# oppo-us-research/PoP-Net

Measured on AMD Instinct MI355X. Metric: depth-frames/sec end-to-end (480x640), higher is better.
Workload: dtype bf16

## Files before the change

### popnet_amd/csrc/api.hip

```cpp
#pragma clang fp contract(off)
#include <cmath>
#include <cstdarg>
#include <cstdio>
#include <cstdlib>
#include <cstring>
#include "pn_internal.h"
#include "preproc_pixel.h"

template <typename TIN>
__global__ void preprocess_kernel(const TIN *__restrict__ depth, float *__restrict__ out, int B, int H, int W, int S,
                                  double scale_x, double scale_y, float dmax, float mean, float stdv) {
    const unsigned pix = blockIdx.x * blockDim.x + threadIdx.x;
    if (pix >= (unsigned)(S * S)) return;
    const int b = blockIdx.y;
    const int dy = (int)(pix / (unsigned)S);
    const int dx = (int)(pix - (unsigned)dy * (unsigned)S);
    const size_t gid = (size_t)b * S * S + pix;

    out[gid] = pn_preproc_pixel(depth + (size_t)b * H * W, H, W, dy, dx, scale_x, scale_y, dmax, mean, stdv);
}

PnSwitches pn_read_switches() {
    auto set = [](const char *name) { return getenv(name) != nullptr; };
    auto num = [](const char *name, int unset) { const char *e = getenv(name); return e ? atoi(e) : unset; };
    auto is = [](const char *name, const char *value) { const char *e = getenv(name); return e && !strcmp(e, value); };
    PnSwitches s;
    s.no_conv3 = set("POPNET_NO_CONV3");
    s.conv3_rpg8 = set("POPNET_CONV3_RPG8");
    s.conv3_pt14 = num("POPNET_CONV3_PT14", 0);
    s.conv3_nbuf2 = set("POPNET_CONV3_NBUF2");
    s.generic_c64_off = num("POPNET_GENERIC_C64", 1) == 0;
    if (set("POPNET_CONV4")) s.conv4 = num("POPNET_CONV4", 0) == 0 ? 0 : 1;
    s.no_mix = set("POPNET_NO_MIX");
    s.no_bblock = set("POPNET_NO_BBLOCK");
    s.bblock_x3 = num("POPNET_BBLOCK_X3", 0) != 0;
    s.bb64_static = set("POPNET_BB64_STATIC");
    s.bb64_halves = num("POPNET_BB64_HALVES", 1) == 2 ? 2 : 1;
    s.no_tailfuse = set("POPNET_NO_TAILFUSE");
    s.no_poolfuse = set("POPNET_NO_POOLFUSE");
    s.no_stempool = set("POPNET_NO_STEMPOOL");
    s.no_embed3 = set("POPNET_NO_EMBED3");
    s.train_x3_wide = set("POPNET_TRAIN_X3_WIDE");
    s.train_wgrad_novec = set("POPNET_TRAIN_WGRAD_NOVEC");
    s.trainx_one_stream = num("POPNET_TRAINX_STREAMS", 0) == 1;
    s.trainx_stem_handover = set("POPNET_TRAINX_STEM_HANDOVER");
    s.trainx_stem_gather = is("POPNET_TRAINX_STEM_FWD", "gather");
    s.trainx_stem_bn_separate = is("POPNET_TRAINX_STEM_BN", "separate");
    s.trainx_stem_depth = num("POPNET_TRAINX_STEM_DEPTH", 2);
    s.trainx_pack_gather = is("POPNET_TRAINX_PACK", "gather");
    s.trainx_legacy_wgrad = is("POPNET_TRAINX_WGRAD", "legacy");
    return s;
}

extern "C" {

int pn_abi_version(void) { return PN_ABI_VERSION; }
int pn_build_experiments(void) { return 0; }

pn_ctx *pn_create(int device_id) {
    pn_ctx *ctx = new pn_ctx();
    ctx->device = device_id;
    int ndev = 0;
    hipError_t e = hipGetDeviceCount(&ndev);
    if (e != hipSuccess || device_id < 0 || device_id >= ndev) {
        char buf[256];
        snprintf(buf, sizeof buf, "pn_create: device %d not available (%d devices, %s)", device_id, ndev,
                 hipGetErrorString(e));
        ctx->err = buf;
        ctx->device = -1;
        return ctx;
    }
    hipDeviceProp_t prop;
    if (hipGetDeviceProperties(&prop, device_id) == hipSuccess) ctx->num_cus = prop.multiProcessorCount;
    return ctx;
}

void pn_destroy(pn_ctx *ctx) {
    if (!ctx) return;
    if (ctx->parse_ws) (void)hipFree(ctx->parse_ws);
    pn_parse_big_free(ctx);
    if (ctx->train_ws) (void)hipFree(ctx->train_ws);
    for (void *p : ctx->train_ws_retired) (void)hipFree(p);
    for (auto &e : ctx->train_packs) (void)hipFree(e.buf);
    if (ctx->train_pack_table) (void)hipFree(ctx->train_pack_table);
    delete ctx;
}

}

int pn_set_error(pn_ctx *ctx, int code, const char *fmt, ...) {
    char buf[1024];
    va_list ap;
    va_start(ap, fmt);
    vsnprintf(buf, sizeof(buf), fmt, ap);
    va_end(ap);
    if (ctx) ctx->err = buf;
    return code;
}

extern "C" {

int pn_last_error(pn_ctx *ctx, char *buf, size_t buf_len) {
    if (!ctx) return 0;
    if (buf && buf_len) {
        size_t n = ctx->err.size() < buf_len - 1 ? ctx->err.size() : buf_len - 1;
        memcpy(buf, ctx->err.data(), n);
        buf[n] = 0;
    }
    return (int)ctx->err.size();
}

int pn_preprocess(pn_ctx *ctx, const void *depth_dev, int depth_dtype, int B, int H, int W, float *out_dev, int S,
                  float depth_max, float depth_mean, float depth_std, void *hip_stream) {
    if (!ctx) return PN_ERR_INVALID;
    if (ctx->device < 0) return pn_set_error(ctx, PN_ERR_STATE, "context has no device");
    if (!depth_dev || !out_dev || B < 1 || H < 2 || W < 2 || S < 1)
        return pn_set_error(ctx, PN_ERR_INVALID, "pn_preprocess: bad arguments");
    if (W == 2 * S && H == 2 * S)
        return pn_set_error(ctx, PN_ERR_UNSUPPORTED, "pn_preprocess: %dx%d -> %d is an exact 2x decimation, where cv2.resize(INTER_LINEAR) runs INTER_AREA instead: not built", W, H, S);
    const double inv_x = (double)S / (double)W, inv_y = (double)S / (double)H;
// ... 35 lines not shown
```

### popnet_amd/csrc/bb64_kernel.h

```cpp
#pragma once
#include "conv3_kernel.h"


#define BB_INQ (12 * 32 * 32)
#define BB_IN (4 * BB_INQ)
#define BB_MIDQ (10 * 32 * 32)
#define BB_MID (4 * BB_MIDQ)
#define BB_ASLOT 4096
#define BB_OFF_MID (2 * BB_IN)
#define BB_OFF_A (BB_OFF_MID + BB_MID)
#define BB_NSLOT 6
#define BB_LDS (BB_OFF_A + BB_NSLOT * BB_ASLOT)
#define BB_BIAS(cv, q) (BB_OFF_MID + (q) * BB_MIDQ + (((cv) + 1) * 32 + 30) * 32)

__host__ __device__ constexpr int bb_item_ks(int n, int PT, bool xch) { return !xch || n < 16 * PT ? n / PT : n - 16 * PT < 4 ? 16 + ((n - 16 * PT) >> 1) : 16 + ((n - 16 * PT) & 1); }
__host__ __device__ constexpr int bb_item_pt(int n, int PT, bool xch) { return !xch || n < 16 * PT ? n % PT : n - 16 * PT < 4 ? (n - 16 * PT) & 1 : (n - 16 * PT) >> 1; }

typedef __attribute__((ext_vector_type(2))) float f32x2;
typedef __attribute__((ext_vector_type(2))) __bf16 bf16x2;
typedef __attribute__((ext_vector_type(2))) short i16x2;
__device__ __forceinline__ unsigned bb_relu_pk(unsigned w) {
    return __builtin_bit_cast(unsigned, __builtin_elementwise_max(__builtin_bit_cast(i16x2, w), i16x2{0, 0}));
}

template <int HV>
__global__ __launch_bounds__((4 * HV + 4) * 64, 1) void bb64_kernel(const BBProblem P) {
    typedef __bf16 T;
    constexpr int CT = 4 / HV, NCW = 4 * HV, NP = CT / 2, PT1 = 5, PT2 = 4, KK = 9, BQ = 6;
    constexpr bool SPLIT = HV == 1;
    constexpr bool XCH = HV == 1;
    constexpr int NKO = XCH ? 16 : 18;
    constexpr int FILL1 = 7, FILL2 = 11;
    extern __shared__ __attribute__((aligned(16))) char smem[];
    const int tid = threadIdx.x;
    const int lane = tid & 63;
    const int wave = __builtin_amdgcn_readfirstlane(tid >> 6);
    const int c = lane & 15, q = lane >> 4;
    const int W = P.W, H = P.H;

    volatile int *s_tile = reinterpret_cast<volatile int *>(smem + BB_OFF_MID + 31 * 32);
    const bool dyn = P.tickets != nullptr;
    auto next_tile = [&](int t, int k) -> int { return dyn ? __builtin_amdgcn_readfirstlane(s_tile[(k + 1) & 3]) : t + (int)gridDim.x; };
    auto next_tile_raw = [&](int t, int k) -> int { return dyn ? s_tile[(k + 1) & 3] : t + (int)gridDim.x; };
    auto tile_geom = [&](int t, int &b, int &oy0, int &ox0, int &R, int &Wc) {
        b = t / P.tiles_per_img;
        const int rem = t - b * P.tiles_per_img;
        const int ty = rem / P.tiles_x, tx = rem - ty * P.tiles_x;
        oy0 = ty * 8; ox0 = tx * P.Wt;
        R = min(8, H - oy0); Wc = min(P.Wt, W - ox0);
    };

    if (wave >= NCW) {
        const int lw = wave - NCW;
        const unsigned lane16 = (unsigned)lane * 16u;
        int t = blockIdx.x;
        if (t >= P.ntiles) return;
        if (lw < 2) {
            const char *wsrc = (const char *)P.wpack + lw * 2048;
            auto dma_a = [&](int kstep) {
                pn_glds16_s<0>(wsrc + (size_t)kstep * BB_ASLOT, lane16, (unsigned)(BB_OFF_A + (kstep % BB_NSLOT) * BB_ASLOT) + (unsigned)__builtin_amdgcn_readfirstlane(lw * 2048));
                pn_glds16_s<0>(wsrc + (size_t)kstep * BB_ASLOT + 1024, lane16, (unsigned)(BB_OFF_A + (kstep % BB_NSLOT) * BB_ASLOT + 1024) + (unsigned)__builtin_amdgcn_readfirstlane(lw * 2048));
            };
            dma_a(0); dma_a(1); dma_a(2); dma_a(3);
            asm volatile("s_waitcnt vmcnt(0)\n\ts_barrier" ::: "memory");
            asm volatile("s_barrier" ::: "memory");
            for (int k = 0; t < P.ntiles; ++k) {
                const int tnx = next_tile_raw(t, k);
#pragma clang loop unroll(full)
                for (int p = 0; p < 18; ++p) {
                    dma_a((2 * p + 4) % 36);
                    dma_a((2 * p + 5) % 36);
                    asm volatile("s_waitcnt vmcnt(2)\n\ts_barrier" ::: "memory");
                    if (p == 8) asm volatile("s_barrier" ::: "memory");
                }
                asm volatile("s_barrier" ::: "memory");
                t = __builtin_amdgcn_readfirstlane(tnx);
            }
            asm volatile("s_waitcnt vmcnt(0)" ::: "memory");
            return;
        }
        auto dma_in = [&](int tt, int buf, int n) {
            int b, oy0, ox0, R, Wc;
            tile_geom(tt, b, oy0, ox0, R, Wc);
            const int qu = n / 12, row = n % 12;
            const int px = lane >> 1;
            const int iy = oy0 - 2 + row, ix = ox0 - 2 + px;
            const size_t frame_b = ((size_t)b * H * W * P.in_cs + P.in_coff) * 2;
            const bool inb = px < Wc + 4 && (unsigned)ix < (unsigned)W && (unsigned)iy < (unsigned)H;
            const unsigned off = inb ? (unsigned)((iy * W + ix) * P.in_cs * 2 + qu * 32 + (lane & 1) * 16) : P.in_zero_off - (unsigned)frame_b;
            pn_glds16_s<0>((const char *)P.in + frame_b, off, (unsigned)__builtin_amdgcn_readfirstlane(buf * BB_IN + qu * BB_INQ + row * 1024));
        };
        const int n0 = (lw - 2) * 24;
        const bool ticketer = dyn && lw == 2 && lane == 0;
        int ticket = 0;
        auto claim = [&]() -> int { return 2 * (int)gridDim.x + atomicAdd(P.tickets, 1); };
        if (ticketer) ticket = t + (int)gridDim.x;
#pragma unroll
        for (int j = 0; j < 24; ++j) dma_in(t, 0, n0 + j);
        asm volatile("s_waitcnt vmcnt(0)" ::: "memory");
        if (ticketer) s_tile[1] = ticket;
        asm volatile("s_waitcnt lgkmcnt(0)\n\ts_barrier" ::: "memory");
        asm volatile("s_barrier" ::: "memory");
        int cur = 0;
        for (int k = 0; t < P.ntiles; ++k) {
            const int tnx = next_tile(t, k);
            const int tn = tnx < P.ntiles ? tnx : t;
// ... 267 lines not shown
```

### popnet_amd/csrc/net_run.hip

```cpp
#include <algorithm>
#include <cstring>
#include "net_internal.h"

namespace pnnet {
int upload_net(pn_net *n) {
    pn_ctx *ctx = n->ctx;
    PN_HIP_CHECK(ctx, hipSetDevice(ctx->device));
    for (auto &b : n->bufs) {
        PN_HIP_CHECK(ctx, hipMalloc(&b.p, b.bytes + 2048));
        PN_HIP_CHECK(ctx, hipMemset(b.p, 0, b.bytes + 2048));
    }
    for (auto &im : n->images) {
        PN_HIP_CHECK(ctx, hipMalloc(&im.dev, im.bytes));
        if (im.host.empty()) PN_HIP_CHECK(ctx, hipMemset(im.dev, 0, im.bytes));
        else PN_HIP_CHECK(ctx, hipMemcpy(im.dev, im.host.data(), im.bytes, hipMemcpyHostToDevice));
    }
    PN_HIP_CHECK(ctx, hipDeviceSynchronize());
    return PN_OK;
}

void release_net(pn_net *n) {
    for (auto &b : n->bufs) if (b.p) (void)hipFree(b.p);
    for (auto &im : n->images) if (im.dev) (void)hipFree(im.dev);
    for (auto &r : n->prof) { (void)hipEventDestroy(r.a); (void)hipEventDestroy(r.b); }
// ... 81 lines not shown
        PN_HIP_CHECK(n->ctx, hipMemcpyAsync(n->dev(st.dev_probs), st.host_probs.data(), st.host_probs.size() * sizeof(ConvProblem),
                                            hipMemcpyHostToDevice, stream));
    }
    n->last_B = B;
    for (int i = 0; i < 4; ++i) n->last_nchw[i] = n->nchw_ptr[i];
    return PN_OK;
}

int profile_step(pn_net *n, const Step &st, int B, hipStream_t stream, ProfRec **out) {
    pn_ctx *ctx = n->ctx;
    if (n->prof_used == n->prof.size()) {
        ProfRec r;
        PN_HIP_CHECK(ctx, hipEventCreate(&r.a));
        PN_HIP_CHECK(ctx, hipEventCreate(&r.b));
        n->prof.push_back(r);
    }
    ProfRec *pr = &n->prof[n->prof_used++];
    const bool conv = st.type == Step::CONV || st.type == Step::BBLOCK;
    pr->kind = conv ? (int)Step::CONV : (int)st.type;
    pr->flops = 0;
    for (int id : st.conv_ids) pr->flops += n->convs[id].flops * B;
    pr->label = conv ? step_label(n, st) : std::string();
    PN_HIP_CHECK(ctx, hipEventRecord(pr->a, stream));
    *out = pr;
    return PN_OK;
}
}

int run_forward(pn_net *n, const float *x, int B, hipStream_t stream, int nsteps) {
    pn_ctx *ctx = n->ctx;
    if (B < 1 || B > n->max_batch) return pn_set_error(ctx, PN_ERR_INVALID, "batch %d outside [1, %d]", B, n->max_batch);
    bool dirty = B != n->last_B;
    for (int i = 0; i < 4; ++i) dirty |= n->nchw_ptr[i] != n->last_nchw[i];
    if (dirty) {
        if (n->locked)
            return pn_set_error(ctx, PN_ERR_STATE, "net is locked at batch %d (pn_net_lock): a forward with another batch size or other output buffers would rewrite descriptors a captured graph still reads", n->last_B);
        if (int rc = refresh_problems(n, B, stream)) return rc;
    }
    if (n->tickets_suspect) {
        for (auto &st : n->steps)
            if (st.type == Step::BBLOCK && st.bb_tickets >= 0) PN_HIP_CHECK(ctx, hipMemsetAsync(n->dev(st.bb_tickets), 0, 256, stream));
        n->tickets_suspect = false;
    }
    for (size_t si = 0; si < n->steps.size(); ++si) {
        if ((int)si == nsteps) break;
        Step &st = n->steps[si];
        int rc = PN_OK;
        ProfRec *pr = nullptr;
        if (n->profiling)
            if (int prc = profile_step(n, st, B, stream, &pr)) return prc;
        if (st.type == Step::STEM) {
            const Buf &ob = n->bufs[st.out_buf];
            const PnFrameSrc *src = n->frame_src.frames ? &n->frame_src : nullptr;
            const float *w = (const float *)n->dev(st.stem_w), *bias = (const float *)n->dev(st.stem_b);
            float *scratch = (float *)n->dev(st.stem_scratch);
            if (st.stem_pool_buf >= 0) {
                const Buf &pb = n->bufs[st.stem_pool_buf];
                rc = pn_launch_stem_pool(ctx, x, n->dev(st.stem_wfrag), bias, pb.p, B, n->in_h, n->in_w, ob.H, ob.W, pb.C, stream, src);
            } else if (st.stem_cin > 1) {
                if (src) return pn_set_error(ctx, PN_ERR_UNSUPPORTED, "the frames-in forward takes single-channel depth frames (input_dim = 1)");
                rc = pn_conv2d_forward(ctx, x, w, bias, scratch, B, st.stem_cin, n->in_h, n->in_w, 64, 7, 2, 3, 0, (void *)stream);
                if (!rc) rc = pn_launch_nchw_relu_to_nhwc(ctx, n->prec, scratch, ob.p, B, ob.H, ob.W, 64, ob.C, n->x3 ? ob.plane : 0, stream);
            } else {
                rc = pn_launch_stem(ctx, n->x3 ? PN_PREC_BF16X3 : n->prec, x, w, n->dev(st.stem_wfrag), bias, ob.p, B, n->in_h, n->in_w, ob.H, ob.W, ob.C, n->x3 ? ob.plane : 0, stream, src);
            }
        } else if (st.type == Step::POOL) {
            const Buf &ib = n->bufs[st.pool.in_buf], &ob = n->bufs[st.pool.out_buf];
            rc = pn_launch_pool(ctx, n->prec, st.pool.mode, ib.p, ob.p, B, ib.H, ib.W, st.pool.C, ib.C, ob.C, st.pool.out_coff, n->x3 ? ib.plane : 0, n->x3 ? ob.plane : 0, stream);
        } else if (st.type == Step::BBLOCK) {
            const ConvSpec &ca = n->convs[st.conv_ids[0]], &cb = n->convs[st.conv_ids[1]];
            const Buf &ib = n->bufs[ca.in_buf], &ob = n->bufs[cb.out_buf];
            BBProblem P;
            memset(&P, 0, sizeof P);
            P.in = ib.p; P.out = ob.p; P.wpack = n->dev(st.bb_wpack); P.bias1 = (const float *)n->dev(st.bb_bias1); P.bias2 = (const float *)n->dev(st.bb_bias2);
            P.B = B; P.H = ib.H; P.W = ib.W;
            P.in_cs = ib.C; P.in_coff = ca.in_coff; P.out_cs = ob.C; P.out_coff = cb.out_coff;
            P.Wt = st.bb_wt; P.tiles_x = (ib.W + st.bb_wt - 1) / st.bb_wt;
            P.tiles_per_img = ((ib.H + (n->x3 ? 5 : 7)) / (n->x3 ? 6 : 8)) * P.tiles_x;
            P.ntiles = B * P.tiles_per_img;
            P.in_zero_off = (unsigned)ib.bytes;
            P.in_split = n->x3 ? ib.plane : 0; P.out_split = n->x3 ? ob.plane : 0;
            P.tickets = (n->x3 || n->sw.bb64_static || P.ntiles < 4 * ctx->num_cus) ? nullptr : (int *)n->dev(st.bb_tickets);
            P.halves = n->sw.bb64_halves;
            rc = n->x3 ? pn_launch_bb64x3(ctx, P, stream) : pn_launch_bb64(ctx, P, stream);
        } else {
            rc = pn_launch_conv(ctx, st.launch, stream);
        }
        if (rc) { n->tickets_suspect = true; return rc; }
        if (pr) PN_HIP_CHECK(ctx, hipEventRecord(pr->b, stream));
    }
    return PN_OK;
}
}

using namespace pnnet;

extern "C" {
int pn_net_profile_begin(pn_net *n) {
    if (!n) return PN_ERR_INVALID;
    n->prof_by_kernel.clear();
    n->profiling = true;
    n->prof_used = 0;
    return PN_OK;
}

int pn_net_profile_end(pn_net *n, double *conv_ms, int64_t *conv_launches, double *conv_flops, double *other_ms,
                       int64_t *other_launches) {
    if (!n) return PN_ERR_INVALID;
    pn_ctx *ctx = n->ctx;
    n->profiling = false;
    ProfRow conv, other;
    for (size_t i = 0; i < n->prof_used; ++i) {
        PN_HIP_CHECK(ctx, hipEventSynchronize(n->prof[i].b));
        float ms = 0.f;
        PN_HIP_CHECK(ctx, hipEventElapsedTime(&ms, n->prof[i].a, n->prof[i].b));
        auto add = [&](ProfRow &r) { r.ms += ms; r.launches += 1; r.flops += n->prof[i].flops; };
        if (n->prof[i].kind == (int)Step::CONV) { add(conv); add(n->prof_by_kernel[n->prof[i].label]); }
        else add(other);
    }
    n->prof_used = 0;
    if (conv_ms) *conv_ms = conv.ms;
    if (conv_launches) *conv_launches = conv.launches;
    if (conv_flops) *conv_flops = conv.flops;
    if (other_ms) *other_ms = other.ms;
    if (other_launches) *other_launches = other.launches;
    return PN_OK;
}

int pn_net_profile_kernel(pn_net *n, int rank, char *name, size_t name_cap, double *ms, int64_t *launches, double *flops) {
    if (!n || rank < 0) return PN_ERR_INVALID;
    std::vector<std::pair<double, std::string>> order;
    for (auto &kv : n->prof_by_kernel) order.push_back({-kv.second.ms, kv.first});
    std::sort(order.begin(), order.end());
    if ((size_t)rank >= order.size()) return PN_ERR_INVALID;
    const ProfRow &e = n->prof_by_kernel[order[rank].second];
    if (name && name_cap) { strncpy(name, order[rank].second.c_str(), name_cap - 1); name[name_cap - 1] = 0; }
    if (ms) *ms = e.ms;
    if (launches) *launches = e.launches;
    if (flops) *flops = e.flops;
    return PN_OK;
}
}
```

### popnet_amd/csrc/pn_internal.h

```cpp
#pragma once
#include <hip/hip_runtime.h>
#include <stdint.h>
#include <string.h>
#include <string>
#include <vector>
#include "../../include/popnet_hip.h"

struct pn_ctx {
    int device = 0;
    std::string err;
    int num_cus = 256;
    void *parse_ws = nullptr;
    size_t parse_ws_bytes = 0;
    bool parse_ws_fixed = false;
    int parse_last_b = 0;
    void *parse_big = nullptr;
    void *train_ws = nullptr;
    size_t train_ws_bytes = 0;
    bool train_ws_keep = false;
    std::vector<void *> train_ws_retired;
    bool train_lds_attr = false;
    bool train_x3 = false;
    struct PackEntry { const float *w; int Cout, Cin, flip, x3; void *buf; size_t bytes; bool fresh; };
    bool train_pack_cache = false;
    std::vector<PackEntry> train_packs;
    void *train_pack_table = nullptr;
    size_t train_pack_table_entries = 0;
    size_t train_pack_table_cap = 0;
    unsigned train_pack_blocks = 0;
};

struct PnSwitches {
    bool no_conv3 = false;
    bool conv3_rpg8 = false;
    int conv3_pt14 = 0;
    bool conv3_nbuf2 = false;
    bool generic_c64_off = false;
    int conv4 = -1;
    bool no_mix = false;
    bool no_bblock = false;
    bool bblock_x3 = false;
    bool bb64_static = false;
    int bb64_halves = 1;
    bool no_tailfuse = false;
    bool no_poolfuse = false;
    bool no_stempool = false;
    bool no_embed3 = false;
    bool train_x3_wide = false;
    bool train_wgrad_novec = false;
    bool trainx_one_stream = false;
    bool trainx_stem_handover = false;
    bool trainx_stem_gather = false;
    bool trainx_stem_bn_separate = false;
    int trainx_stem_depth = 2;
    bool trainx_pack_gather = false;
    bool trainx_legacy_wgrad = false;
};
PnSwitches pn_read_switches();

int pn_set_error(pn_ctx *ctx, int code, const char *fmt, ...);

inline uint16_t pn_f32_to_bf16(float f) {
    uint32_t u;
    memcpy(&u, &f, 4);
    if ((u & 0x7fffffffu) > 0x7f800000u) return (uint16_t)((u >> 16) | 0x40);
    u += 0x7fffu + ((u >> 16) & 1u);
    return (uint16_t)(u >> 16);
}
inline float pn_bf16_to_f32(uint16_t h) { const uint32_t u = (uint32_t)h << 16; float f; memcpy(&f, &u, 4); return f; }
void pn_parse_big_free(pn_ctx *ctx);
int pn_train_ws(pn_ctx *ctx, size_t bytes, void **out);
const char *pn_dgrad_strided_plan(int N, int Cin, int H, int W, int ks, unsigned *grid_x, unsigned *grid_y);

#define PN_HIP_CHECK(ctx, expr)                                                              \
    do {                                                                                     \
        hipError_t _e = (expr);                                                              \
        if (_e != hipSuccess)                                                                \
            return pn_set_error((ctx), PN_ERR_HIP, "%s failed: %s (%s:%d)", #expr,           \
                                hipGetErrorString(_e), __FILE__, __LINE__);                  \
    } while (0)

struct PnLdsAttr { size_t bytes[64] = {}; };
inline int pn_lds_attr(pn_ctx *ctx, PnLdsAttr &st, const void *kern, size_t bytes) {
    const int d = ctx->device >= 0 && ctx->device < 64 ? ctx->device : 0;
    if (st.bytes[d] >= bytes) return PN_OK;
    PN_HIP_CHECK(ctx, hipFuncSetAttribute(kern, hipFuncAttributeMaxDynamicSharedMemorySize, (int)bytes));
    st.bytes[d] = bytes;
    return PN_OK;
}

enum pn_act {
    PN_ACT_NONE = 0,
    PN_ACT_RELU = 1,
    PN_ACT_LEAKY = 2,
    PN_ACT_SIG_PM2 = 3,
    PN_ACT_SIG = 4,
    PN_ACT_YOLO = 5
};

struct ConvProblem {
    const void *in;
    const void *wpack;
    const float *bias;
    const void *res;
    void *out;
    float *out_nchw;
    int B, H, W;
    int Ho, Wo;
    int cin_chunks;
    int in_cs, in_coff;
    int cout;
    int out_cs, out_coff;
    int res_cs, res_coff;
    int act;
    int yolo_naf;
    int R;
    int Wt, tiles_x;
    int tiles_per_img;
    int cout_blocks;
    int nblocks;
    int ksteps;
    int ks;
    int lds_buf_bytes;
    int lds_two;
    unsigned in_zero_off;
    int split;
    int res_split;
    int in_wrap;
    const void *tail_w;
    const float *tail_bias;
    void *tail_out;
    float *tail_nchw;
    int tail_cout, tail_act, tail_out_cs, tail_out_coff;
    int tail_split;
};

enum pn_conv_cfg {
    PN_CFG_C128 = 0,
    PN_CFG_C64 = 1,
    PN_CFG_C32 = 2,
    PN_CFG_C16 = 3,
    PN_CFG_C64W = 4
};
int pn_cfg_couts(int cfg);
inline int pn_cfg_ct(int cfg) { return cfg == PN_CFG_C16 ? 1 : 2; }
inline int pn_conv_row_channel(int tile, int row, int CT) {
    return (tile / CT) * CT * 16 + 4 * CT * (row >> 2) + 4 * (tile % CT) + (row & 3);
}
int pn_cfg_pixels(int cfg);

struct ConvLaunch {
    int prec;
    int ks;
    int stride;
    int pitch;
    int cfg;
    int kern = 0, wc = 0, wp = 0, nbuf = 0, pt = 7, rpg = 4;
    int dil = 1;
    int acc = 0;
    int tail = 0;
    int mix = 0;
    int nprob;
    int max_blocks;
    size_t lds_bytes;
    const ConvProblem *probs_dev;
};
int pn_launch_conv(pn_ctx *ctx, const ConvLaunch &L, hipStream_t stream);
inline std::string pn_conv_kernel_label(int prec, int kern, bool mix, int ks, int stride, int pitch, int cfg, int wc, int wp, int nbuf, int pt, int rpg) {
    char lb[96];
    if (kern == 4) snprintf(lb, sizeof lb, "conv4_kernel");
    else if (kern == 3 && mix) snprintf(lb, sizeof lb, "conv3_mix_kernel");
    else if (kern == 3) snprintf(lb, sizeof lb, "conv3_kernel<%d, %d, %d, %d, %d, %d>", ks, wc, wp, nbuf, pt, rpg);
    else snprintf(lb, sizeof lb, "conv_mfma_kernel<%d, %d, %d, %d, %d>", prec, ks, stride, pitch, cfg);
    return lb;
}
inline std::string pn_conv_kernel_label_dil(int prec, int ks, int stride, int pitch, int cfg, int dil) {
    char lb[96];
    snprintf(lb, sizeof lb, "conv_mfma_kernel<%d, %d, %d, %d, %d, %d>", prec, ks, stride, pitch, cfg, dil);
    return lb;
}
inline std::string pn_pool_kernel_label(int mode, bool split) {
    char lb[48];
    snprintf(lb, sizeof lb, "pool_kernel<%d%s>", mode, split ? ", split" : "");
    return lb;
}
int pn_launch_conv3(pn_ctx *ctx, const ConvLaunch &L, hipStream_t stream);
int pn_launch_conv4(pn_ctx *ctx, const ConvLaunch &L, hipStream_t stream);

struct BBProblem {
    const void *in;
    void *out;
    const void *wpack;
    const float *bias1, *bias2;
    int B, H, W;
    int in_cs, in_coff, out_cs, out_coff;
    int Wt, tiles_x, tiles_per_img, ntiles;
    unsigned in_zero_off;
    int in_split, out_split;
    int *tickets;
    int halves;
};
int pn_launch_bb64(pn_ctx *ctx, const BBProblem &P, hipStream_t stream);
int pn_launch_bb64x3(pn_ctx *ctx, const BBProblem &P, hipStream_t stream);
size_t pn_conv3_lds_bytes(int ks, int WP, int nbuf, int rpg = 4);
size_t pn_conv_lds_bytes(int prec, int ks, int stride, int pitch, int R, int dil = 1);
int pn_conv_has_instance_d2(int prec, int ks, int stride, int pitch, int cfg);
constexpr size_t PN_CONV_LDS_MAX = 160 * 1024;
int pn_conv_stage_maxpx(int prec, int ks, int stride, int pitch, int cfg);

struct PnFrameSrc;
int pn_launch_stem_pool(pn_ctx *ctx, const float *x, const void *wfrag, const float *bias, void *out, int B, int H, int W, int Ho, int Wo,
                        int out_cs, hipStream_t stream, const PnFrameSrc *src);
struct PnFrameSrc;
int pn_launch_stem(pn_ctx *ctx, int prec, const float *x, const float *w, const void *wfrag, const float *bias,
                   void *out, int B, int H, int W, int Ho, int Wo, int out_cs, int split, hipStream_t stream, const PnFrameSrc *src = nullptr);

int pn_launch_pool(pn_ctx *ctx, int prec, int mode, const void *in, void *out, int B, int H, int W,
                   int C, int in_cs, int out_cs, int out_coff, int in_split, int out_split, hipStream_t stream);

int pn_stem_forward_planes(pn_ctx *ctx, const float *x_dev, const float *w_dev, void *y_planes, int cs, int split, int f32, int N, int Cin, int H, int W, int Cout,
                           int ks, int stride, int pad, int gather, hipStream_t s);
struct PnStemBn {
    const void *x; int x_cs, x_split;
    const float *mean, *invstd, *k1, *k2, *k3, *scale, *shift;
    int act;
};
int pn_stem_wgrad_planes(pn_ctx *ctx, const float *x_dev, const void *dy_planes, int cs, int split, int f32, const PnStemBn *bn, float *dw_dev, int N, int Cin, int H,
                         int W, int Cout, int ks, int stride, int pad, int depth, hipStream_t s);
int pn_launch_nchw_relu_to_nhwc(pn_ctx *ctx, int prec, const float *in, void *out, int B, int H, int W, int C, int out_cs, int split, hipStream_t stream);
int pn_launch_nhwc_to_nchw(pn_ctx *ctx, int prec, const void *in, float *out, int B, int H, int W,
                           int C, int in_cs, int in_coff, int split, hipStream_t stream);
```

Before: 69580.

## Add strip-scheduled fused basic-block kernel reusing conv1 halo rows between vertical tiles

Adds a new bb64s strip kernel in which each workgroup walks a vertical strip of 8-row tiles. It carries the last conv1 output rows over to the next tile through an LDS copy, so subsequent tiles compute only the new rows (PT1=4 instead of 5). This removes halo recomputation in the first conv and amortizes weight streaming across consecutive tiles. The host picks the strip count from the CU count, and the kernel is enabled by default when enough row tiles exist. In exchange it shortens per-workgroup parallelism, adds serial dependence along strips, and adds extra ticket and barrier logic.

```diff
diff --git a/popnet_amd/csrc/api.hip b/popnet_amd/csrc/api.hip
--- a/popnet_amd/csrc/api.hip
+++ b/popnet_amd/csrc/api.hip
@@ -36,6 +36,7 @@
     s.bblock_x3 = num("POPNET_BBLOCK_X3", 0) != 0;
     s.bb64_static = set("POPNET_BB64_STATIC");
     s.bb64_halves = num("POPNET_BB64_HALVES", 1) == 2 ? 2 : 1;
+    if (set("POPNET_BB64_STRIP")) { const int v = num("POPNET_BB64_STRIP", 0); s.bb64_strip = v == 1 || v == 2 ? v : 0; }
     s.no_tailfuse = set("POPNET_NO_TAILFUSE");
     s.no_poolfuse = set("POPNET_NO_POOLFUSE");
     s.no_stempool = set("POPNET_NO_STEMPOOL");
diff --git a/popnet_amd/csrc/bb64_common.h b/popnet_amd/csrc/bb64_common.h
--- /dev/null
+++ b/popnet_amd/csrc/bb64_common.h
@@ -0,0 +1,24 @@
+#pragma once
+#include "conv3_kernel.h"
+
+
+#define BB_INQ (12 * 32 * 32)
+#define BB_IN (4 * BB_INQ)
+#define BB_MIDQ (10 * 32 * 32)
+#define BB_MID (4 * BB_MIDQ)
+#define BB_ASLOT 4096
+#define BB_OFF_MID (2 * BB_IN)
+#define BB_OFF_A (BB_OFF_MID + BB_MID)
+#define BB_NSLOT 6
+#define BB_LDS (BB_OFF_A + BB_NSLOT * BB_ASLOT)
+#define BB_BIAS(cv, q) (BB_OFF_MID + (q) * BB_MIDQ + (((cv) + 1) * 32 + 30) * 32)
+
+__host__ __device__ constexpr int bb_item_ks(int n, int PT, bool xch) { return !xch || n < 16 * PT ? n / PT : n - 16 * PT < 4 ? 16 + ((n - 16 * PT) >> 1) : 16 + ((n - 16 * PT) & 1); }
+__host__ __device__ constexpr int bb_item_pt(int n, int PT, bool xch) { return !xch || n < 16 * PT ? n % PT : n - 16 * PT < 4 ? (n - 16 * PT) & 1 : (n - 16 * PT) >> 1; }
+
+typedef __attribute__((ext_vector_type(2))) float f32x2;
+typedef __attribute__((ext_vector_type(2))) __bf16 bf16x2;
+typedef __attribute__((ext_vector_type(2))) short i16x2;
+__device__ __forceinline__ unsigned bb_relu_pk(unsigned w) {
+    return __builtin_bit_cast(unsigned, __builtin_elementwise_max(__builtin_bit_cast(i16x2, w), i16x2{0, 0}));
+}
diff --git a/popnet_amd/csrc/bb64_kernel.h b/popnet_amd/csrc/bb64_kernel.h
--- a/popnet_amd/csrc/bb64_kernel.h
+++ b/popnet_amd/csrc/bb64_kernel.h
@@ -1,27 +1,6 @@
 #pragma once
-#include "conv3_kernel.h"
-
-
-#define BB_INQ (12 * 32 * 32)
-#define BB_IN (4 * BB_INQ)
-#define BB_MIDQ (10 * 32 * 32)
-#define BB_MID (4 * BB_MIDQ)
-#define BB_ASLOT 4096
-#define BB_OFF_MID (2 * BB_IN)
-#define BB_OFF_A (BB_OFF_MID + BB_MID)
-#define BB_NSLOT 6
-#define BB_LDS (BB_OFF_A + BB_NSLOT * BB_ASLOT)
-#define BB_BIAS(cv, q) (BB_OFF_MID + (q) * BB_MIDQ + (((cv) + 1) * 32 + 30) * 32)
-
-__host__ __device__ constexpr int bb_item_ks(int n, int PT, bool xch) { return !xch || n < 16 * PT ? n / PT : n - 16 * PT < 4 ? 16 + ((n - 16 * PT) >> 1) : 16 + ((n - 16 * PT) & 1); }
-__host__ __device__ constexpr int bb_item_pt(int n, int PT, bool xch) { return !xch || n < 16 * PT ? n % PT : n - 16 * PT < 4 ? (n - 16 * PT) & 1 : (n - 16 * PT) >> 1; }
-
-typedef __attribute__((ext_vector_type(2))) float f32x2;
-typedef __attribute__((ext_vector_type(2))) __bf16 bf16x2;
-typedef __attribute__((ext_vector_type(2))) short i16x2;
-__device__ __forceinline__ unsigned bb_relu_pk(unsigned w) {
-    return __builtin_bit_cast(unsigned, __builtin_elementwise_max(__builtin_bit_cast(i16x2, w), i16x2{0, 0}));
-}
+#include "bb64_common.h"
+
 
 template <int HV>
 __global__ __launch_bounds__((4 * HV + 4) * 64, 1) void bb64_kernel(const BBProblem P) {
diff --git a/popnet_amd/csrc/bb64s_inst.hip b/popnet_amd/csrc/bb64s_inst.hip
--- /dev/null
+++ b/popnet_amd/csrc/bb64s_inst.hip
@@ -0,0 +1,3 @@
+#include "bb64s_kernel.h"
+
+int pn_launch_bb64s(pn_ctx *ctx, const BBProblem &P, hipStream_t stream) { return bb64s_launch(ctx, P, ctx->num_cus, stream); }
diff --git a/popnet_amd/csrc/bb64s_kernel.h b/popnet_amd/csrc/bb64s_kernel.h
--- /dev/null
+++ b/popnet_amd/csrc/bb64s_kernel.h
@@ -0,0 +1,375 @@
+#pragma once
+#include <type_traits>
+#include "bb64_common.h"
+
+__global__ __launch_bounds__(512, 1) void bb64s_strip_kernel(const BBProblem P) {
+    constexpr int CT = 4, NCW = 4, NP = 2, PT2 = 4, KK = 9, BQ = 6, NKO = 16;
+    constexpr int FILL1 = 7, FILL2 = 11;
+    extern __shared__ __attribute__((aligned(16))) char smem[];
+    const int tid = threadIdx.x;
+    const int lane = tid & 63;
+    const int wave = __builtin_amdgcn_readfirstlane(tid >> 6);
+    const int c = lane & 15, q = lane >> 4;
+    const int W = P.W, H = P.H;
+    const int nseg = P.nseg, grid = (int)gridDim.x;
+
+    volatile int *s_next = reinterpret_cast<volatile int *>(smem + BB_OFF_MID + 31 * 32);
+    const bool dyn = P.tickets != nullptr;
+    auto next_seg_raw = [&](int seg) -> int { return dyn ? s_next[0] : seg + grid; };
+    auto seg_geom = [&](int seg, int &b, int &ox0, int &Wc, int &ty0, int &len) {
+        const int col = seg / P.strip_S, si = seg - col * P.strip_S;
+        b = col / P.tiles_x;
+        const int tx = col - b * P.tiles_x;
+        ox0 = tx * P.Wt; Wc = min(P.Wt, W - ox0);
+        const int base = P.strip_T / P.strip_S, rem = P.strip_T - base * P.strip_S;
+        ty0 = si * base + min(si, rem);
+        len = base + (si < rem ? 1 : 0);
+    };
+
+    int seg = blockIdx.x;
+    if (seg >= nseg) return;
+    int sb_, sox0, sWc, sty0, slen, j = 0;
+    seg_geom(seg, sb_, sox0, sWc, sty0, slen);
+
+    if (wave >= NCW) {
+        const int lw = wave - NCW;
+        const unsigned lane16 = (unsigned)lane * 16u;
+        if (lw < 2) {
+            const char *wsrc = (const char *)P.wpack + lw * 2048;
+            auto dma_a = [&](int kstep) {
+                pn_glds16_s<0>(wsrc + (size_t)kstep * BB_ASLOT, lane16, (unsigned)(BB_OFF_A + (kstep % BB_NSLOT) * BB_ASLOT) + (unsigned)__builtin_amdgcn_readfirstlane(lw * 2048));
+                pn_glds16_s<0>(wsrc + (size_t)kstep * BB_ASLOT + 1024, lane16, (unsigned)(BB_OFF_A + (kstep % BB_NSLOT) * BB_ASLOT + 1024) + (unsigned)__builtin_amdgcn_readfirstlane(lw * 2048));
+            };
+            dma_a(0); dma_a(1); dma_a(2); dma_a(3);
+            asm volatile("s_waitcnt vmcnt(0)\n\ts_barrier" ::: "memory");
+            asm volatile("s_barrier" ::: "memory");
+            while (seg < nseg) {
+                const int snx = next_seg_raw(seg);
+#pragma clang loop unroll(full)
+                for (int p = 0; p < 18; ++p) {
+                    dma_a((2 * p + 4) % 36);
+                    dma_a((2 * p + 5) % 36);
+                    asm volatile("s_waitcnt vmcnt(2)\n\ts_barrier" ::: "memory");
+                    if (p == 8) asm volatile("s_barrier" ::: "memory");
+                }
+                asm volatile("s_barrier" ::: "memory");
+                if (++j == slen) {
+                    seg = __builtin_amdgcn_readfirstlane(snx);
+                    j = 0;
+                    seg_geom(seg, sb_, sox0, sWc, sty0, slen);
+                }
+            }
+            asm volatile("s_waitcnt vmcnt(0)" ::: "memory");
+            return;
+        }
+        auto dma_in = [&](int b, int oy0, int ox0, int Wc, int buf, int n) {
+            const int qu = n / 12, row = n % 12;
+            const int px = lane >> 1;
+            const int iy = oy0 - 2 + row, ix = ox0 - 2 + px;
+            const size_t frame_b = ((size_t)b * H * W * P.in_cs + P.in_coff) * 2;
+            const bool inb = px < Wc + 4 && (unsigned)ix < (unsigned)W && (unsigned)iy < (unsigned)H;
+            const unsigned off = inb ? (unsigned)((iy * W + ix) * P.in_cs * 2 + qu * 32 + (lane & 1) * 16) : P.in_zero_off - (unsigned)frame_b;
+            pn_glds16_s<0>((const char *)P.in + frame_b, off, (unsigned)__builtin_amdgcn_readfirstlane(buf * BB_IN + qu * BB_INQ + row * 1024));
+        };
+        const int n0 = (lw - 2) * 24;
+        const bool ticketer = dyn && lw == 2 && lane == 0;
+        int ticket = 0;
+        int cpy[4];
+#pragma unroll
+        for (int n = 0; n < 4; ++n) {
+            const int i = (lw - 2) * 64 + lane + 128 * n;
+            const int qp = i / 120, r = (i - qp * 120) / 60, w = i - qp * 120 - r * 60;
+            cpy[n] = i < 480 ? BB_OFF_MID + qp * BB_MIDQ + (8 + r) * 1024 + w * 16 : -1;
+        }
+#pragma unroll
+        for (int n = 0; n < 24; ++n) dma_in(sb_, sty0 * 8, sox0, sWc, 0, n0 + n);
+        asm volatile("s_waitcnt vmcnt(0)" ::: "memory");
+        asm volatile("s_barrier" ::: "memory");
+        asm volatile("s_barrier" ::: "memory");
+        int cur = 0;
+        while (seg < nseg) {
+            if (j > 0) {
+                u32x4 v[4];
+#pragma unroll
+                for (int n = 0; n < 4; ++n)
+                    if (cpy[n] >= 0) v[n] = *reinterpret_cast<const u32x4 *>(smem + cpy[n]);
+#pragma unroll
+                for (int n = 0; n < 4; ++n)
+                    if (cpy[n] >= 0) *reinterpret_cast<u32x4 *>(smem + cpy[n] - 8 * 1024) = v[n];
+                asm volatile("s_waitcnt lgkmcnt(0)" ::: "memory");
+            }
+            const bool lastj = j == slen - 1;
+            int nsg = seg, nb = sb_, nox0 = sox0, nWc = sWc, nty0 = sty0, nlen = slen, nj = j + 1;
+            if (lastj) {
+                nsg = __builtin_amdgcn_readfirstlane(next_seg_raw(seg));
+                nj = 0;
+                if (nsg < nseg) seg_geom(nsg, nb, nox0, nWc, nty0, nlen);
+                else nj = j;
+            }
+            const int noy0 = (nty0 + nj) * 8;
+            int signed_off = -1;
+            if (ticketer) {
+                if (j == 0) ticket = grid + atomicAdd(P.tickets, 1);
+                else if (j == 1 && ticket >= nseg) signed_off = atomicAdd(P.tickets + 1, 1);
+            }
+#pragma clang loop unroll(full)
+            for (int p = 0; p < 18; ++p) {
+                if (p < 12) { dma_in(nb, noy0, nox0, nWc, cur ^ 1, n0 + 2 * p); dma_in(nb, noy0, nox0, nWc, cur ^ 1, n0 + 2 * p + 1); }
+                asm volatile("s_barrier" ::: "memory");
+                if (p == 8) asm volatile("s_barrier" ::: "memory");
+            }
+            asm volatile("s_waitcnt vmcnt(0)" ::: "memory");
+            if (ticketer) {
+                if (j == 0) s_next[0] = ticket;
+                if (signed_off == grid - 1) {
+                    __hip_atomic_store(P.tickets, 0, __ATOMIC_RELAXED, __HIP_MEMORY_SCOPE_AGENT);
+                    __hip_atomic_store(P.tickets + 1, 0, __ATOMIC_RELAXED, __HIP_MEMORY_SCOPE_AGENT);
+                }
+            }
+            asm volatile("s_waitcnt lgkmcnt(0)\n\ts_barrier" ::: "memory");
+            cur ^= 1;
+            if (lastj) { seg = nsg; sb_ = nb; sox0 = nox0; sWc = nWc; sty0 = nty0; slen = nlen; j = 0; }
+            else j = nj;
+        }
+        return;
+    }
+
+    const int pw = wave;
+    if (wave == 0) {
+        *reinterpret_cast<float *>(smem + BB_BIAS(0, q) + c * 4) = P.bias1[lane];
+        *reinterpret_cast<float *>(smem + BB_BIAS(1, q) + c * 4) = P.bias2[lane];
+    }
+    const int h = pw & 1;
+    auto pct = [&](int i) -> int { return i ^ (2 * h); };
+    auto pc = [&](int k) -> int { return k ^ h; };
+    const int biasaddr = BB_BIAS(0, q);
+    float b1[4 * CT], b2[4 * CT];
+    int aaddr0 = BB_OFF_A + lane * 16 + pct(0) * 1024, aaddr1 = aaddr0 ^ 2048;
+    asm volatile("" : "+v"(aaddr0), "+v"(aaddr1));
+    bf16x8 aq[2][CT], bq[BQ];
+    asm volatile("s_barrier" ::: "memory");
+#pragma unroll
+    for (int ct = 0; ct < CT; ++ct) aq[0][ct] = *reinterpret_cast<const bf16x8 *>(smem + (ct < 2 ? aaddr0 : aaddr1) + (ct & 1) * 1024);
+    asm volatile("s_waitcnt lgkmcnt(0)\n\ts_barrier" ::: "memory");
+    int cur = 0;
+    while (seg < nseg) {
+        const int snx = next_seg_raw(seg);
+        const int b = sb_, ox0 = sox0, Wc = sWc, oy0 = (sty0 + j) * 8, R = min(8, H - oy0);
+        const int MC = Wc + 2, nout = R * Wc;
+        const float inv_mc = 1.0f / (float)MC, inv_wc = 1.0f / (float)Wc;
+        const int inb = cur * BB_IN;
+        auto out_tile = [&](int pt) -> int { return pt < 3 ? pw * 3 + pt : 12 + (pw >> 1); };
+        int cc = c;
+        asm volatile("" : "+v"(cc));
+        const float fc = (float)cc + 0.5f;
+        const int ba1base = inb + (q >> 1) * BB_INQ + (q & 1) * 16, ba2base = BB_OFF_MID + (q >> 1) * BB_MIDQ + (q & 1) * 16;
+        const int dumppix = (3 * 32 + 30 + (cc & 1)) * 32;
+        int ba2[PT2];
+#pragma unroll
+        for (int pt = 0; pt < PT2; ++pt) {
+            const int sb = out_tile(pt) * 16, s = sb + cc;
+            const int r = (int)((fc + (float)sb) * inv_wc), x = s - r * Wc;
+            ba2[pt] = ba2base + (s < nout ? (r * 32 + x) * 32 : 0);
+        }
+        f32x4 acc[CT][5];
+        const bool border = oy0 == 0 || ox0 == 0 || oy0 + R >= H || ox0 + Wc >= W;
+        const int midw = BB_OFF_MID + q * BB_MIDQ + 16 * pc(0);
+#define BB_TAPOFF(tap) ((((tap) / 3) * 32 + ((tap) % 3)) * 32)
+#define BB_A(k, ct) (*reinterpret_cast<const bf16x8 *>(smem + ((ct) < 2 ? aaddr0 : aaddr1) + ((k) % BB_NSLOT) * BB_ASLOT + ((ct) & 1) * 1024))
+#define BB_KOFF1(ks) (((ks) / KK) * 2 * BB_INQ + BB_TAPOFF((ks) % KK))
+#define BB_B1(n) (*reinterpret_cast<const bf16x8 *>(smem + ba1[bb_item_pt(n, PT1, true)] + BB_KOFF1(bb_item_ks(n, PT1, true))))
+        auto conv1 = [&](auto pt1c) __attribute__((always_inline)) {
+            constexpr int PT1 = decltype(pt1c)::value;
+            constexpr int ROW0 = PT1 == 5 ? 0 : 2;
+            const int nmid = (R + 2 - ROW0) * MC;
+            int ba1[PT1];
+#pragma unroll
+            for (int pt = 0; pt < PT1; ++pt) {
+                const int sb = (pw * PT1 + pt) * 16, s = sb + cc;
+                const int r = (int)((fc + (float)sb) * inv_mc), x = s - r * MC;
+                ba1[pt] = ba1base + (s < nmid ? ((r + ROW0) * 32 + x) * 32 : dumppix);
+            }
+#pragma unroll
+            for (int ct = 0; ct < CT; ++ct)
+#pragma unroll
+                for (int pt = 0; pt < PT1; ++pt) acc[ct][pt] = f32x4{0.f, 0.f, 0.f, 0.f};
+            auto epi1 = [&](int pt) {
+                const int pix = ba1[pt] - ba1base, r = pix >> 10, x = (pix >> 5) & 31;
+                const bool inside = (unsigned)(oy0 - 1 + r) < (unsigned)H && (unsigned)(ox0 - 1 + x) < (unsigned)W;
+                const unsigned keep = !border || inside ? 0xffffffffu : 0u;
+                u32x4 o[NP];
+#pragma unroll
+                for (int ct = 0; ct < CT; ++ct) {
+                    f32x2 lo = {acc[ct][pt][0] + b1[4 * ct + 0], acc[ct][pt][1] + b1[4 * ct + 1]};
+                    f32x2 hi = {acc[ct][pt][2] + b1[4 * ct + 2], acc[ct][pt][3] + b1[4 * ct + 3]};
+                    o[ct >> 1][2 * (ct & 1)] = bb_relu_pk(__builtin_bit_cast(unsigned, __builtin_convertvector(lo, bf16x2))) & keep;
+                    o[ct >> 1][2 * (ct & 1) + 1] = bb_relu_pk(__builtin_bit_cast(unsigned, __builtin_convertvector(hi, bf16x2))) & keep;
+                }
+                const int dsta = midw + pix;
+                *reinterpret_cast<u32x4 *>(smem + dsta) = o[0];
+                *reinterpret_cast<u32x4 *>(smem + (dsta ^ 16)) = o[1];
+            };
+#pragma unroll
+            for (int n = 0; n < BQ - 1; ++n) bq[n] = BB_B1(n);
+#pragma clang loop unroll(full)
+            for (int ph = 0; ph < NKO; ++ph) {
+                __builtin_amdgcn_sched_barrier(0);
+#pragma clang loop unroll(full)
+                for (int pt = 0; pt < PT1; ++pt) {
+                    const int n = ph * PT1 + pt, nr = n + BQ - 1;
+                    if (pt < CT) aq[(ph + 1) & 1][pt] = BB_A(ph + 1, pt);
+                    if (nr < 18 * PT1) bq[nr % BQ] = BB_B1(nr);
+#pragma unroll
+                    for (int ct = 0; ct < CT; ++ct)
+                        acc[ct][pt] = __builtin_amdgcn_mfma_f32_16x16x32_bf16(aq[ph & 1][ct], bq[n % BQ], acc[ct][pt], 0, 0, 0);
+                    if (pt < CT && nr < 18 * PT1) __builtin_amdgcn_sched_group_barrier(0x100, 2, 0);
+                    else if (pt < CT || nr < 18 * PT1) __builtin_amdgcn_sched_group_barrier(0x100, 1, 0);
+                    __builtin_amdgcn_sched_group_barrier(0x008, CT, 0);
+                }
+                __builtin_amdgcn_sched_barrier(0);
+                if (ph & 1) asm volatile("s_barrier" ::: "memory");
+            }
+#pragma unroll
+            for (int i = 0; i < CT; ++i) *reinterpret_cast<f32x4 *>(b1 + 4 * i) = *reinterpret_cast<const f32x4 *>(smem + biasaddr + 16 * pct(i));
+            __builtin_amdgcn_sched_barrier(0);
+#pragma unroll
+            for (int ct = 0; ct < CT; ++ct) aq[1][ct] = BB_A(17, ct);
+#pragma clang loop unroll(full)
+            for (int m = 0; m < 2 * PT1; ++m) {
+                const int n = 16 * PT1 + m, nr = n + BQ - 1, pt = bb_item_pt(n, PT1, true), ks = bb_item_ks(n, PT1, true);
+                if (nr < 18 * PT1) bq[nr % BQ] = BB_B1(nr);
+#pragma unroll
+                for (int ct = 0; ct < CT; ++ct)
+                    acc[ct][pt] = __builtin_amdgcn_mfma_f32_16x16x32_bf16(aq[ks & 1][ct], bq[n % BQ], acc[ct][pt], 0, 0, 0);
+                if (m == 2 * PT1 - 2) {
+#pragma unroll
+                    for (int ct = 0; ct < CT; ++ct) aq[0][ct] = BB_A(18, ct);
+                }
+                if (ks == 17 && pt < PT1 - 1) epi1(pt);
+                if (m == 0) __builtin_amdgcn_sched_group_barrier(0x100, CT + 1, 0);
+                else if (nr < 18 * PT1) __builtin_amdgcn_sched_group_barrier(0x100, 1, 0);
+#pragma unroll
+                for (int ct = 0; ct < CT; ++ct) {
+                    __builtin_amdgcn_sched_group_barrier(0x008, 1, 0);
+                    if (m >= 3) __builtin_amdgcn_sched_group_barrier(0x206, FILL1, 0);
+                }
+                if (m == 2 * PT1 - 2) __builtin_amdgcn_sched_group_barrier(0x100, CT, 0);
+            }
+            __builtin_amdgcn_sched_barrier(0);
+            asm volatile("s_barrier" ::: "memory");
+            epi1(PT1 - 1);
+        };
+        if (j == 0) conv1(std::integral_constant<int, 5>());
+        else conv1(std::integral_constant<int, 4>());
+        asm volatile("s_waitcnt lgkmcnt(0)\n\ts_barrier" ::: "memory");
+        const int resw = inb + q * BB_INQ + (2 * 32 + 2) * 32 + 16 * pc(0);
+        __amdgpu_buffer_rsrc_t orsrc;
+        auto epi2 = [&](int pt) {
+            const int nct = pt == 3 ? 2 : CT, np = nct / 2;
+            const int pix = ba2[pt] - ba2base, r = pix >> 10, x = (pix >> 5) & 31;
+            const bool valid = out_tile(pt) * 16 + cc < nout;
+            u32x4 rr[NP], o[NP];
+            rr[0] = *reinterpret_cast<const u32x4 *>(smem + resw + pix);
+            if (np == 2) rr[NP - 1] = *reinterpret_cast<const u32x4 *>(smem + ((resw + pix) ^ 16));
+#pragma unroll
+            for (int ct = 0; ct < nct; ++ct) {
+                const unsigned ra = rr[ct >> 1][2 * (ct & 1)], rb = rr[ct >> 1][2 * (ct & 1) + 1];
+                f32x2 lo = {acc[ct][pt][0] + b2[4 * ct + 0] + __builtin_bit_cast(float, ra << 16),
+                            acc[ct][pt][1] + b2[4 * ct + 1] + __builtin_bit_cast(float, ra & 0xffff0000u)};
+                f32x2 hi = {acc[ct][pt][2] + b2[4 * ct + 2] + __builtin_bit_cast(float, rb << 16),
+                            acc[ct][pt][3] + b2[4 * ct + 3] + __builtin_bit_cast(float, rb & 0xffff0000u)};
+                o[ct >> 1][2 * (ct & 1)] = bb_relu_pk(__builtin_bit_cast(unsigned, __builtin_convertvector(lo, bf16x2)));
+                o[ct >> 1][2 * (ct & 1) + 1] = bb_relu_pk(__builtin_bit_cast(unsigned, __builtin_convertvector(hi, bf16x2)));
+            }
+            unsigned vin = (unsigned)(((oy0 + r) * W + ox0 + x) * P.out_cs * 2 + 32 * q);
+            asm volatile("" : "+v"(vin));
+            const unsigned voff = valid ? vin : 0x80000000u;
+#pragma unroll
+            for (int k = 0; k < np; ++k) __builtin_amdgcn_raw_buffer_store_b128(o[k], orsrc, voff + 16u * (unsigned)pc(k), 0, 0);
+        };
+#define BB_KOFF2(ks) (((ks) / KK) * 2 * BB_MIDQ + BB_TAPOFF((ks) % KK))
+#define BB_B2(n) (*reinterpret_cast<const bf16x8 *>(smem + ba2[bb_item_pt(n, PT2, true)] + BB_KOFF2(bb_item_ks(n, PT2, true))))
+#pragma unroll
+        for (int ct = 0; ct < CT; ++ct)
+#pragma unroll
+            for (int pt = 0; pt < PT2; ++pt) acc[ct][pt] = f32x4{0.f, 0.f, 0.f, 0.f};
+#pragma unroll
+        for (int n = 0; n < BQ - 1; ++n) bq[n] = BB_B2(n);
+#pragma clang loop unroll(full)
+        for (int p2 = 0; p2 < NKO; ++p2) {
+            const int ph = 18 + p2;
+            __builtin_amdgcn_sched_barrier(0);
+#pragma clang loop unroll(full)
+            for (int pt = 0; pt < PT2; ++pt) {
+                const int n = p2 * PT2 + pt, nr = n + BQ - 1;
+                if (pt < CT) aq[(ph + 1) & 1][pt] = BB_A(ph + 1, pt);
+                if (nr < 18 * PT2) bq[nr % BQ] = BB_B2(nr);
+                const int nct = pt == 3 ? 2 : CT;
+#pragma unroll
+                for (int ct = 0; ct < nct; ++ct)
+                    acc[ct][pt] = __builtin_amdgcn_mfma_f32_16x16x32_bf16(aq[ph & 1][ct], bq[n % BQ], acc[ct][pt], 0, 0, 0);
+                if (pt < CT && nr < 18 * PT2) __builtin_amdgcn_sched_group_barrier(0x100, 2, 0);
+                else if (pt < CT || nr < 18 * PT2) __builtin_amdgcn_sched_group_barrier(0x100, 1, 0);
+                if (pt == 3) __builtin_amdgcn_sched_group_barrier(0x008, 2, 0);
+                else __builtin_amdgcn_sched_group_barrier(0x008, CT, 0);
+            }
+            __builtin_amdgcn_sched_barrier(0);
+            if (ph & 1) asm volatile("s_barrier" ::: "memory");
+        }
+#pragma unroll
+        for (int i = 0; i < CT; ++i) *reinterpret_cast<f32x4 *>(b2 + 4 * i) = *reinterpret_cast<const f32x4 *>(smem + biasaddr + 1024 + 16 * pct(i));
+        orsrc = __builtin_amdgcn_make_buffer_rsrc((char *)P.out + ((size_t)b * H * W * P.out_cs + P.out_coff) * 2, 0, (int)((size_t)H * W * P.out_cs * 2), 0x00020000);
+        __builtin_amdgcn_sched_barrier(0);
+#pragma unroll
+        for (int ct = 0; ct < CT; ++ct) aq[1][ct] = BB_A(35, ct);
+#pragma clang loop unroll(full)
+        for (int m = 0; m < 2 * PT2; ++m) {
+            const int n = 16 * PT2 + m, nr = n + BQ - 1, pt = bb_item_pt(n, PT2, true), ks = bb_item_ks(n, PT2, true);
+            const int nct = pt == 3 ? 2 : CT;
+            if (nr < 18 * PT2) bq[nr % BQ] = BB_B2(nr);
+#pragma unroll
+            for (int ct = 0; ct < nct; ++ct)
+                acc[ct][pt] = __builtin_amdgcn_mfma_f32_16x16x32_bf16(aq[ks & 1][ct], bq[n % BQ], acc[ct][pt], 0, 0, 0);
+            if (m == 2 * PT2 - 2) {
+#pragma unroll
+                for (int ct = 0; ct < CT; ++ct) aq[0][ct] = BB_A(36, ct);
+            }
+            if (ks == 17 && pt < PT2 - 1) epi2(pt);
+            if (m == 0) __builtin_amdgcn_sched_group_barrier(0x100, CT + 1, 0);
+            else if (nr < 18 * PT2) __builtin_amdgcn_sched_group_barrier(0x100, 1, 0);
+#pragma unroll
+            for (int ct = 0; ct < nct; ++ct) {
+                __builtin_amdgcn_sched_group_barrier(0x008, 1, 0);
+                if (m >= 3) __builtin_amdgcn_sched_group_barrier(0x146, FILL2, 0);
+            }
+            if (m == 2 * PT2 - 2) __builtin_amdgcn_sched_group_barrier(0x100, CT, 0);
+        }
+        __builtin_amdgcn_sched_barrier(0);
+        asm volatile("s_barrier" ::: "memory");
+        epi2(PT2 - 1);
+        asm volatile("s_waitcnt lgkmcnt(0)\n\ts_barrier" ::: "memory");
+        cur ^= 1;
+        if (++j == slen) {
+            seg = __builtin_amdgcn_readfirstlane(snx);
+            j = 0;
+            seg_geom(seg, sb_, sox0, sWc, sty0, slen);
+        }
+    }
+#undef BB_A
+#undef BB_B1
+#undef BB_B2
+#undef BB_KOFF1
+#undef BB_KOFF2
+#undef BB_TAPOFF
+}
+
+static int bb64s_launch(pn_ctx *ctx, const BBProblem &P, int num_cus, hipStream_t stream) {
+    static PnLdsAttr attr;
+    if (P.strip_S < 1 || P.strip_T < 2 * P.strip_S || P.nseg != P.B * P.tiles_x * P.strip_S)
+        return pn_set_error(ctx, PN_ERR_INVALID, "bb64s: %d segments per column of %d row tiles (every segment needs two tiles)", P.strip_S, P.strip_T);
+    if (int rc = pn_lds_attr(ctx, attr, reinterpret_cast<const void *>(bb64s_strip_kernel), BB_LDS)) return rc;
+    const int grid = P.nseg < num_cus ? P.nseg : num_cus;
+    hipLaunchKernelGGL(bb64s_strip_kernel, dim3(grid), dim3(512), BB_LDS, stream, P);
+    PN_HIP_CHECK(ctx, hipGetLastError());
+    return PN_OK;
+}
diff --git a/popnet_amd/csrc/net_run.hip b/popnet_amd/csrc/net_run.hip
--- a/popnet_amd/csrc/net_run.hip
+++ b/popnet_amd/csrc/net_run.hip
@@ -187,7 +187,15 @@
             P.in_split = n->x3 ? ib.plane : 0; P.out_split = n->x3 ? ob.plane : 0;
             P.tickets = (n->x3 || n->sw.bb64_static || P.ntiles < 4 * ctx->num_cus) ? nullptr : (int *)n->dev(st.bb_tickets);
             P.halves = n->sw.bb64_halves;
-            rc = n->x3 ? pn_launch_bb64x3(ctx, P, stream) : pn_launch_bb64(ctx, P, stream);
+            const int T = (ib.H + 7) / 8, ncols = B * P.tiles_x;
+            int S = std::max(1, std::min((ctx->num_cus + ncols - 1) / ncols, T / 2));
+            if (n->sw.bb64_strip == 2) S = std::max(1, std::min(2 * S, T / 2));
+            const bool strip = !n->x3 && T >= 2 && (n->sw.bb64_strip >= 1 || (n->sw.bb64_strip < 0 && !n->sw.bb64_static && n->sw.bb64_halves != 2 && T >= 4 * S));
+            if (strip) {
+                P.strip_S = S; P.strip_T = T; P.nseg = ncols * S;
+                P.tickets = (n->sw.bb64_static || P.nseg <= ctx->num_cus) ? nullptr : (int *)n->dev(st.bb_tickets);
+            }
+            rc = n->x3 ? pn_launch_bb64x3(ctx, P, stream) : strip ? pn_launch_bb64s(ctx, P, stream) : pn_launch_bb64(ctx, P, stream);
         } else {
             rc = pn_launch_conv(ctx, st.launch, stream);
         }
diff --git a/popnet_amd/csrc/pn_internal.h b/popnet_amd/csrc/pn_internal.h
--- a/popnet_amd/csrc/pn_internal.h
+++ b/popnet_amd/csrc/pn_internal.h
@@ -42,6 +42,7 @@
     bool bblock_x3 = false;
     bool bb64_static = false;
     int bb64_halves = 1;
+    int bb64_strip = -1;
     bool no_tailfuse = false;
     bool no_poolfuse = false;
     bool no_stempool = false;
@@ -199,8 +200,10 @@
     int in_split, out_split;
     int *tickets;
     int halves;
+    int strip_S, strip_T, nseg;
 };
 int pn_launch_bb64(pn_ctx *ctx, const BBProblem &P, hipStream_t stream);
+int pn_launch_bb64s(pn_ctx *ctx, const BBProblem &P, hipStream_t stream);
 int pn_launch_bb64x3(pn_ctx *ctx, const BBProblem &P, hipStream_t stream);
 size_t pn_conv3_lds_bytes(int ks, int WP, int nbuf, int rpg = 4);
 size_t pn_conv_lds_bytes(int prec, int ks, int stride, int pitch, int R, int dil = 1);
```

New measurement: 70600, median of 6. +1.5%, better.
